# kristi700/ViT-SSL

Hardware: AMD Instinct MI355X
Metric: images_per_sec (higher is better)
Workload: dtype bf16; 1 GPU; ViT-B/16 SimMIM 224x224 mask 0.6 dropout 0.1 AdamW, batch 256/GPU; global_batch=256, parallelism=dp1

## Files before the change

__graft_entry__.py:

```python
import os
import subprocess
import sys
from concurrent.futures import ThreadPoolExecutor

ROOT = os.path.dirname(os.path.abspath(__file__))
PKG = os.path.join(ROOT, "vit-ssl_amd")
CSRC = os.path.join(PKG, "csrc")
OUT_DIR = os.path.join(PKG, "vitssl_hip")
LIB = os.path.join(OUT_DIR, "libvitssl_hip.so")
SOURCES = ["error.cpp", "gemm_nt.hip", "gemm_tn.hip", "layernorm.hip", "attention.hip", "attention_hd.hip", "elementwise.hip", "patch.hip", "dino.hip", "augment.hip", "transforms.hip", "metrics.hip", "classify.hip", "mixup.hip", "fp8.hip", "optim.hip", "droppath.hip", "layerscale.hip", "lamb.hip"]
HIPCC = os.environ.get("HIPCC", "/opt/rocm/bin/hipcc")
PER_FILE_FLAGS = {"augment.hip": ["-ffp-contract=off"], "transforms.hip": ["-ffp-contract=off"]}
FLAGS = ["--offload-arch=gfx950", "-O3", "-fPIC", "-std=c++17", "-Wno-unused-result"] + os.environ.get("VITSSL_HIPCC_FLAGS", "").split()


def _needs_rebuild(target, deps):
    if not os.path.exists(target):
        return True
    t = os.path.getmtime(target)
    return any(os.path.getmtime(d) > t for d in deps if os.path.exists(d))


def build(force: bool = False, verbose: bool = False) -> None:
    srcs = [os.path.join(CSRC, s) for s in SOURCES if os.path.exists(os.path.join(CSRC, s))]
    hdrs = [os.path.join(CSRC, "common.h"), os.path.join(CSRC, "attention_tiles.h"), os.path.join(CSRC, "attention_bwd.h"),
            os.path.join(CSRC, "resample_taps.h"),
            os.path.join(ROOT, "include", "vitssl_hip.h"), os.path.join(ROOT, "include", "vitssl_transforms.h"),
            os.path.join(ROOT, "include", "vitssl_metrics.h"), os.path.join(ROOT, "include", "vitssl_classify.h"),
            os.path.join(ROOT, "include", "vitssl_attention_hd.h"), os.path.join(ROOT, "include", "vitssl_patch.h"),
            os.path.join(ROOT, "include", "vitssl_optim.h"), os.path.join(ROOT, "include", "vitssl_mixup.h"),
            os.path.join(ROOT, "include", "vitssl_droppath.h"), os.path.join(ROOT, "include", "vitssl_layerscale.h"),
            os.path.join(ROOT, "include", "vitssl_lamb.h"), os.path.join(ROOT, "include", "vitssl_bce.h")]
    objdir = os.path.join(CSRC, "build")
    os.makedirs(objdir, exist_ok=True)

    def compile_one(src):
        obj = os.path.join(objdir, os.path.basename(src) + ".o")
        if force or _needs_rebuild(obj, [src] + hdrs + [os.path.abspath(__file__)]):
            cmd = [HIPCC] + FLAGS + PER_FILE_FLAGS.get(os.path.basename(src), []) + ["-x", "hip", "-c", src, "-o", obj]
            r = subprocess.run(cmd, capture_output=True, text=True)
            if r.returncode != 0:
                raise RuntimeError(f"hipcc failed for {src}:\n{r.stderr[-4000:]}")
            if verbose and r.stderr.strip():
                print(r.stderr, file=sys.stderr)
        return obj

    with ThreadPoolExecutor(max_workers=4) as ex:
        objs = list(ex.map(compile_one, srcs))
    if force or _needs_rebuild(LIB, objs):
# ... 24 lines not shown
```

vit-ssl_amd/csrc/gemm_tn.hip:

```cpp
#include <stdlib.h>
#include <type_traits>
#include "common.h"

#ifdef VITSSL_TN_STAMPS
__device__ unsigned long long* g_tn_stamps = nullptr;
extern "C" int vitssl_debug_set_tn_stamps(unsigned long long* p) {
  return hipMemcpyToSymbol(HIP_SYMBOL(g_tn_stamps), &p, sizeof(p)) == hipSuccess ? 0 : 1;
}
#endif

namespace {

constexpr int TN_T = 256;
constexpr int TN_KM = 64;
constexpr int TN8_KM = 128;
constexpr int TN_THREADS = 512;
constexpr int TN_TILE_BYTES = TN_KM * TN_T * 2;
constexpr int TN_LDS_BYTES = 4 * TN_TILE_BYTES;

struct TnPtr {
  const void* p;
  __host__ __device__ operator const bf16_t*() const { return (const bf16_t*)p; }
  __host__ __device__ operator const unsigned char*() const { return (const unsigned char*)p; }
};

struct TnParams {
  TnPtr A, B;
  float* C;
  long long M;
  int N1, N2;
  int tiles1, tiles2, splits;
  int chunks_per_split;
  float* slabs;
  int direct;
  const float* alpha;
  const float* alpha2;
};

// ... 184 lines not shown
    return;
  }
#pragma unroll
  for (int i = 0; i < 8; ++i) {
    const int n1 = c1 + w1 * 128 + i * 16 + (lane & 15);
    if (n1 >= p.N1) continue;
#pragma unroll
    for (int j = 0; j < 4; ++j) {
      const int n2 = c2 + w2 * 64 + j * 16 + 4 * (lane >> 4);
      if (n2 >= p.N2) continue;
      float* q = p.dst + (long long)n1 * p.N2 + n2;
      if (p.mode == 0) {
        *(f32x4*)q = acc[i][j];
      } else if (p.mode == 1) {
        *(f32x4*)q = *(const f32x4*)q + acc[i][j];
      } else {
#pragma unroll
        for (int r = 0; r < 4; ++r) unsafeAtomicAdd(q + r, acc[i][j][r]);
      }
    }
  }
}

constexpr int TN_MAX_JOBS = 8;
struct TnBatchParams {
  const void* A[TN_MAX_JOBS];
  const void* B[TN_MAX_JOBS];
  float* C[TN_MAX_JOBS];
  int N1[TN_MAX_JOBS], N2[TN_MAX_JOBS];
  int tiles2[TN_MAX_JOBS];
  int tile0[TN_MAX_JOBS + 1];
  int njobs;
  long long M;
  int splits, chunks_per_split;
  int rem_chunks;
  float* slots;
};

struct TnBatchWalk {
  int first, step, end;
};
__device__ __forceinline__ TnBatchWalk tn_batch_walk(const TnBatchParams& p) {
  const int G = gridDim.x;
  const int bid = xcd_remap(blockIdx.x, G);
  const int T = p.tile0[p.njobs];
  const int mainu = T * p.splits;
  TnBatchWalk w;
  if (p.rem_chunks > 0) {
    if (bid < mainu) {
      w.first = bid;
      w.step = mainu + T;
      w.end = mainu;
    } else {
      w.first = mainu + (bid - mainu);
      w.step = G - mainu;
      w.end = mainu + T;
    }
  } else {
    w.first = bid;
    w.step = G;
    w.end = mainu;
  }
  return w;
}
__device__ __forceinline__ void tn_batch_unit(const TnBatchParams& p, int un, int km, int& j, int& c1, int& c2, long long& ch_begin, int& nk) {
  const int T = p.tile0[p.njobs];
  const int split = un / T;
  const int gt = un - split * T;
  j = 0;
#pragma unroll
  for (int q = 1; q < TN_MAX_JOBS; ++q)
    if (q < p.njobs && gt >= p.tile0[q]) j = q;
  const int lt = gt - p.tile0[j];
  const int t1 = lt / p.tiles2[j], t2 = lt - t1 * p.tiles2[j];
  c1 = t1 * TN_T;
  c2 = t2 * TN_T;
  const long long total_chunks = (p.M + km - 1) / km;
  ch_begin = (long long)split * p.chunks_per_split;
  long long ch_end = split < p.splits ? ch_begin + p.chunks_per_split : total_chunks;
  if (ch_end > total_chunks) ch_end = total_chunks;
  nk = ch_begin < ch_end ? (int)(ch_end - ch_begin) : 0;
}

struct Tn8BatchParams {
  TnBatchParams b;
  const float* alpha[TN_MAX_JOBS];
  const float* alpha2[TN_MAX_JOBS];
};
template <class P>
__host__ __device__ __forceinline__ auto& tn_base(P& pp) {
  if constexpr (std::is_same_v<std::remove_const_t<P>, Tn8BatchParams>) return pp.b;
  else return pp;
}
__device__ __forceinline__ void tn_job_scalars(const TnBatchParams&, int, TnUnit& u) { u.alpha = u.alpha2 = nullptr; }
__device__ __forceinline__ void tn_job_scalars(const Tn8BatchParams& p, int j, TnUnit& u) {
  u.alpha = p.alpha[j];
  u.alpha2 = p.alpha2[j];
}

__global__ __launch_bounds__(256) void tn_batch_reduce_kernel(TnBatchParams p) {
  const int T = p.tile0[p.njobs];
  const int gt = blockIdx.x >> 3, rblk = blockIdx.x & 7;
  int j = 0;
  for (int q = 1; q < p.njobs; ++q)
    if (gt >= p.tile0[q]) j = q;
  const int lt = gt - p.tile0[j];
  const int t1 = lt / p.tiles2[j], t2 = lt - t1 * p.tiles2[j];
  const int col = 4 * (threadIdx.x & 63);
  const int n2 = t2 * TN_T + col;
  if (n2 >= p.N2[j]) return;
#pragma unroll 2
  for (int r = threadIdx.x >> 6; r < 32; r += 4) {
    const int row = rblk * 32 + r;
    const int n1 = t1 * TN_T + row;
    if (n1 >= p.N1[j]) break;
    float* q = p.C[j] + (long long)n1 * p.N2[j] + n2;
    f32x4 a = *(const f32x4*)q;
    const float* sl = p.slots + (long long)gt * (TN_T * TN_T) + row * TN_T + col;
    const long long sstride = (long long)T * (TN_T * TN_T);
    const int nsl = p.splits + (p.rem_chunks > 0 ? 1 : 0);
    int s = 0;
    for (; s + 4 <= nsl; s += 4) {
      const f32x4 v0 = *(const f32x4*)(sl + (s + 0) * sstride), v1 = *(const f32x4*)(sl + (s + 1) * sstride);
      const f32x4 v2 = *(const f32x4*)(sl + (s + 2) * sstride), v3 = *(const f32x4*)(sl + (s + 3) * sstride);
      a += (v0 + v1) + (v2 + v3);
    }
    for (; s < nsl; ++s) a += *(const f32x4*)(sl + s * sstride);
    *(f32x4*)q = a;
  }
}

__device__ __forceinline__ int tn8_f(int row) { return (row & 7) | (((row >> 5) & 1) << 3); }

__device__ __forceinline__ int tn8_fa(int row) { return ((row >> 1) & 3) | (((row >> 5) & 1) << 2); }

__device__ __forceinline__ void tn8_pp_unit(const TnUnit& p, char* smem) {
  constexpr int AG = TN8_KM * 128;
  constexpr int BT = TN8_KM * 256;
  constexpr int B_BASE = 4 * AG;
  constexpr unsigned OOBV = 0x80000000u;
  const int lane = threadIdx.x & 63;
  const int wave = __builtin_amdgcn_readfirstlane(threadIdx.x >> 6);
  const int w1 = wave >> 2, w2 = wave & 3;
  const int c1 = p.c1, c2 = p.c2;
  const long long ch_begin = p.ch_begin;
  const int nk = p.nk;

  auto window = [&](const unsigned char* base, int ncols, int t) {
    const long long row0 = (ch_begin + t) * (long long)TN8_KM;
    const long long rows = t < nk ? p.M - row0 : 0;
    return __builtin_amdgcn_make_buffer_rsrc((void*)(base + row0 * ncols), 0, (int)(rows * ncols), 0x00020000);
  };
// ... 207 lines not shown
  F::unit(u, smem);
  F::hand_over();
}

__global__ __launch_bounds__(TN_THREADS, 2) void gemm_tn_pp_kernel(TnParams p) {
  extern __shared__ __attribute__((aligned(16))) char smem[];
  tn_single_body<TnBf16>(p, smem);
}
__global__ __launch_bounds__(TN_THREADS, 2) void gemm_tn_fp8_kernel(TnParams p) {
  extern __shared__ __attribute__((aligned(16))) char smem[];
  tn_single_body<TnFp8>(p, smem);
}
__global__ __launch_bounds__(TN_THREADS, 2) void gemm_tn_batch_kernel(TnBatchParams p) {
  extern __shared__ __attribute__((aligned(16))) char smem[];
  const TnBatchWalk w = tn_batch_walk(tn_base(p));
  for (int un = w.first; un < w.end; un += w.step) tn_batch_step<TnBf16>(p, un, smem);
}
__global__ __launch_bounds__(TN_THREADS, 2) void gemm_tn_fp8_batch_kernel(Tn8BatchParams p) {
  extern __shared__ __attribute__((aligned(16))) char smem[];
  const TnBatchWalk w = tn_batch_walk(tn_base(p));
  for (int un = w.first; un < w.end; un += w.step) tn_batch_step<TnFp8>(p, un, smem);
}

__global__ void tn_reduce_kernel(float* __restrict__ C, const float* __restrict__ slabs, long long n4, long long stride, int splits) {
  for (long long i = (long long)blockIdx.x * blockDim.x + threadIdx.x; i < n4; i += (long long)gridDim.x * blockDim.x) {
    f32x4 a = *(const f32x4*)(C + 4 * i);
    for (int s = 0; s < splits; ++s) a += *(const f32x4*)(slabs + s * stride + 4 * i);
    *(f32x4*)(C + 4 * i) = a;
  }
}

int tn_reduce_slabs(float* C, const float* slabs, int N1, int N2, int splits, hipStream_t s, const char* who) {
  const long long n4 = (long long)N1 * N2 / 4;
  long long grid = (n4 + 255) / 256;
  if (grid > 2048) grid = 2048;
  hipLaunchKernelGGL(tn_reduce_kernel, dim3((unsigned)grid), dim3(256), 0, s, C, slabs, n4, (long long)N1 * N2, splits);
  VS_CHECK_LAUNCH(who);
  return VITSSL_OK;
}

void tn_plan(long long M, int N1, int N2, int* tiles1, int* tiles2, int* splits, int* chunks_per_split, int km = TN_KM) {
  *tiles1 = (N1 + TN_T - 1) / TN_T;
  *tiles2 = (N2 + TN_T - 1) / TN_T;
  const long long total_chunks = (M + km - 1) / km;
  const int ntiles = *tiles1 * *tiles2;
  long long sp = vitssl_persistent_cus() / ntiles;
  if (sp < 1) sp = 1;
  if (sp > total_chunks) sp = total_chunks;
  *chunks_per_split = (int)((total_chunks + sp - 1) / sp);
  *splits = (int)((total_chunks + *chunks_per_split - 1) / *chunks_per_split);
}

void tn_batch_plan(long long M, int T, int G, int* splits, int* chunks_per_split, int* rem_chunks, int km = TN_KM) {
  const long long total_chunks = (M + km - 1) / km;
  const double c_kt = 1.46, c_unit = 9.0, c_part = 0.15;
  double best = 1e30;
  int best_s = 1;
  const long long smax = total_chunks < 64 ? total_chunks : 64;
  for (long long sp = 1; sp <= smax; ++sp) {
    const long long cps = (total_chunks + sp - 1) / sp;
    const long long s_eff = (total_chunks + cps - 1) / cps;
    if (s_eff != sp) continue;
    const long long units = (long long)T * sp;
    const long long rounds = (units + G - 1) / G;
    const double cost = (double)rounds * ((double)cps * c_kt + c_unit) + (sp > 1 ? (double)units * c_part : 0.0);
    if (cost < best) {
      best = cost;
      best_s = (int)sp;
    }
  }
  static VsEnvInt forced_env;
  const int forced = forced_env.get("VITSSL_TN_BATCH_SPLITS", 0);
  if (forced > 0 && forced <= total_chunks) best_s = forced;
  *chunks_per_split = (int)((total_chunks + best_s - 1) / best_s);
  *splits = (int)((total_chunks + *chunks_per_split - 1) / *chunks_per_split);
  *rem_chunks = 0;
  static VsEnvInt rem_env;
  const int use_rem = rem_env.get("VITSSL_TN_BATCH_REM", 1);
  const long long mainu = (long long)T * *splits;
  const long long R = G - mainu;
  if (use_rem && mainu <= G && R >= 8) {
    const double c_rem = 2.2;
    const long long S = *splits;
    const double nr = (double)((T + R - 1) / R);
    const double L = (nr * ((double)total_chunks * c_rem + c_unit) - c_unit) / (c_kt + nr * (double)S * c_rem);
    long long Li = (long long)(L + 0.999);
    const long long rem = total_chunks - S * Li;
    const double t_main = (double)Li * c_kt + c_unit, t_rem = nr * ((double)rem * c_rem + c_unit);
    const double t_old = (double)*chunks_per_split * c_kt + c_unit;
    const double tax = (double)T * c_part * (S == 1 ? 2.0 : 1.0);
    if (rem >= 4 && Li >= 4 && (t_main > t_rem ? t_main : t_rem) + tax < 0.95 * t_old) {
      *chunks_per_split = (int)Li;
      *rem_chunks = (int)rem;
    }
  }
}
long long tn_batch_need(int splits, int rem_chunks, int T) {
  return (splits > 1 || rem_chunks > 0) ? (long long)(splits + (rem_chunks > 0)) * T * TN_T * TN_T : 0;
}

void tn_fill_operands(TnBatchParams& p, int j, const vitssl_tn_job_t* q) {
  p.A[j] = q ? q->A : nullptr;
  p.B[j] = q ? q->B : nullptr;
}
void tn_fill_operands(Tn8BatchParams& p, int j, const vitssl_fp8_tn_job_t* q) {
  p.b.A[j] = q ? q->A8 : nullptr;
  p.b.B[j] = q ? q->B8 : nullptr;
  p.alpha[j] = q ? q->alpha : nullptr;
  p.alpha2[j] = q ? q->alpha2 : nullptr;
}
template <class Params, class Job>
int tn_batch_fill(const Job* jobs, int njobs, Params* pp) {
  TnBatchParams& p = tn_base(*pp);
  int t = 0;
  for (int j = 0; j < TN_MAX_JOBS; ++j) {
    const Job* q = j < njobs ? jobs + j : nullptr;
    tn_fill_operands(*pp, j, q);
    p.C[j] = q ? q->C : nullptr;
    p.N1[j] = q ? q->N1 : 0;
    p.N2[j] = q ? q->N2 : 0;
    p.tile0[j] = t;
// ... 3 lines not shown
  p.tile0[TN_MAX_JOBS] = t;
  p.njobs = njobs;
  return t;
}

template <class F>
int tn_check_operands(const void* A, const void* B, const float* C, long long M, int N1, int N2, int job) {
  char who[48];
  if (job < 0) snprintf(who, sizeof who, "%s", F::NAME);
  else snprintf(who, sizeof who, "%s: job %d", F::BATCH, job);
  VS_CHECK_ARG(A && B && C, "%s: null operand", who);
  VS_CHECK_ARG(job >= 0 || (M > 0 && N1 > 0 && N2 > 0), "%s: empty problem", who);
  VS_CHECK_ARG(N1 > 0 && N2 > 0 && N1 % F::COLS == 0 && N2 % F::COLS == 0, "%s: N1=%d N2=%d must be %smultiples of %d", who, N1, N2,
               job < 0 ? "" : "positive ", F::COLS);
  VS_CHECK_ARG((unsigned long long)M * N1 * F::ESZ < (1ull << 31) && (unsigned long long)M * N2 * F::ESZ < (1ull << 31),
               "%s: operand larger than 2 GiB", who);
  return VITSSL_OK;
}

template <class F>
int64_t tn_single_workspace(int64_t M, int N1, int N2) {
  if (M <= 0 || N1 <= 0 || N2 <= 0) return 0;
  int t1, t2, sp, cps;
  tn_plan(M, N1, N2, &t1, &t2, &sp, &cps, F::KM);
  return (int64_t)sp * N1 * N2;
}

template <class F, void (*KERNEL)(TnParams)>
int tn_launch_single(const void* A, const void* B, float* C, int64_t M, int N1, int N2, const float* alpha, const float* alpha2,
                     float* workspace, int64_t workspace_floats, void* stream) {
  if (int rc = tn_check_operands<F>(A, B, C, M, N1, N2, -1)) return rc;
  TnParams p;
  p.A = {A};
  p.B = {B};
  p.C = C;
  p.M = M;
  p.N1 = N1;
  p.N2 = N2;
  p.alpha = alpha;
  p.alpha2 = alpha2;
  tn_plan(M, N1, N2, &p.tiles1, &p.tiles2, &p.splits, &p.chunks_per_split, F::KM);
  const long long need = (long long)p.splits * N1 * N2;
  p.slabs = (workspace && workspace_floats >= need) ? workspace : nullptr;
  VS_CHECK_ARG(!workspace || p.slabs, "%s: workspace too small (%lld < %lld floats, vitssl_%s_workspace_floats)", F::NAME,
               (long long)workspace_floats, need, F::NAME);
  p.direct = p.splits == 1;
  if (p.direct) p.slabs = nullptr;
  static VsOnce attr_done{false};
  if (int rc = ensure_lds(KERNEL, TN_LDS_BYTES, attr_done, F::NAME)) return rc;
  hipStream_t s = (hipStream_t)stream;
  hipLaunchKernelGGL(KERNEL, dim3(p.tiles1 * p.tiles2 * p.splits), dim3(TN_THREADS), TN_LDS_BYTES, s, p);
  VS_CHECK_LAUNCH(F::NAME);
  return p.slabs ? tn_reduce_slabs(C, p.slabs, N1, N2, p.splits, s, F::REDUCE) : VITSSL_OK;
}

template <class F, class Job>
int64_t tn_batch_workspace(const Job* jobs, int njobs, int64_t M) {
  if (!jobs || njobs <= 0 || njobs > TN_MAX_JOBS || M <= 0) return 0;
  typename F::BatchParams pp;
  const int T = tn_batch_fill(jobs, njobs, &pp);
  int sp, cps, rem;
  tn_batch_plan(M, T, vitssl_persistent_cus(), &sp, &cps, &rem, F::KM);
  return tn_batch_need(sp, rem, T);
}

template <class F, void (*KERNEL)(typename F::BatchParams), class Job>
int tn_launch_batch(const Job* jobs, int njobs, int64_t M, float* workspace, int64_t workspace_floats, void* stream) {
  VS_CHECK_ARG(jobs && njobs > 0 && njobs <= TN_MAX_JOBS, "%s: 1..%d jobs", F::BATCH, TN_MAX_JOBS);
  VS_CHECK_ARG(M > 0, "%s: empty problem", F::BATCH);
  typename F::BatchParams pp;
  TnBatchParams& p = tn_base(pp);
  const int T = tn_batch_fill(jobs, njobs, &pp);
  for (int j = 0; j < njobs; ++j)
    if (int rc = tn_check_operands<F>(p.A[j], p.B[j], p.C[j], M, p.N1[j], p.N2[j], j)) return rc;
  p.M = M;
  const long long cus = vitssl_persistent_cus();
  tn_batch_plan(M, T, (int)cus, &p.splits, &p.chunks_per_split, &p.rem_chunks, F::KM);
  const long long need = tn_batch_need(p.splits, p.rem_chunks, T);
  VS_CHECK_ARG(need == 0 || (workspace && workspace_floats >= need), "%s: workspace of %lld floats needed with %lld CUs available (vitssl_%s_workspace_floats; the answer\n"
               "changes with vitssl_set_reserved_cus: query again after changing the reserve)", F::BATCH, need, cus, F::BATCH);
  p.slots = need ? workspace : nullptr;
  static VsOnce attr_done{false};
  if (int rc = ensure_lds(KERNEL, TN_LDS_BYTES, attr_done, F::BATCH)) return rc;
  hipStream_t s = (hipStream_t)stream;
  const long long units = (long long)T * p.splits;
  const unsigned grid = (unsigned)((units < cus && p.rem_chunks == 0) ? units : cus);
  hipLaunchKernelGGL(KERNEL, dim3(grid), dim3(TN_THREADS), TN_LDS_BYTES, s, pp);
  VS_CHECK_LAUNCH(F::BATCH);
  if (p.slots) {
    hipLaunchKernelGGL(tn_batch_reduce_kernel, dim3((unsigned)T * 8u), dim3(256), 0, s, p);
    VS_CHECK_LAUNCH(F::BATCH_REDUCE);
  }
  return VITSSL_OK;
}

}

extern "C" int64_t vitssl_gemm_tn_workspace_floats(int64_t M, int N1, int N2) { return tn_single_workspace<TnBf16>(M, N1, N2); }
extern "C" int64_t vitssl_gemm_fp8_tn_workspace_floats(int64_t M, int N1, int N2) { return tn_single_workspace<TnFp8>(M, N1, N2); }

extern "C" int vitssl_gemm_bf16_tn(const void* A, const void* B, float* C, int64_t M, int N1, int N2, float* workspace,
                                   int64_t workspace_floats, void* stream) {
  return tn_launch_single<TnBf16, gemm_tn_pp_kernel>(A, B, C, M, N1, N2, nullptr, nullptr, workspace, workspace_floats, stream);
}
extern "C" int vitssl_gemm_fp8_tn(const void* A8, const void* B8, float* C, int64_t M, int N1, int N2, const float* alpha,
                                  const float* alpha2, float* workspace, int64_t workspace_floats, void* stream) {
  return tn_launch_single<TnFp8, gemm_tn_fp8_kernel>(A8, B8, C, M, N1, N2, alpha, alpha2, workspace, workspace_floats, stream);
}

extern "C" int64_t vitssl_gemm_tn_batch_workspace_floats(const vitssl_tn_job_t* jobs, int njobs, int64_t M) {
  return tn_batch_workspace<TnBf16>(jobs, njobs, M);
}
extern "C" int64_t vitssl_gemm_fp8_tn_batch_workspace_floats(const vitssl_fp8_tn_job_t* jobs, int njobs, int64_t M) {
  return tn_batch_workspace<TnFp8>(jobs, njobs, M);
}

extern "C" int vitssl_gemm_bf16_tn_batch(const vitssl_tn_job_t* jobs, int njobs, int64_t M, float* workspace, int64_t workspace_floats,
                                         void* stream) {
  return tn_launch_batch<TnBf16, gemm_tn_batch_kernel>(jobs, njobs, M, workspace, workspace_floats, stream);
}
extern "C" int vitssl_gemm_fp8_tn_batch(const vitssl_fp8_tn_job_t* jobs, int njobs, int64_t M, float* workspace, int64_t workspace_floats,
                                        void* stream) {
  return tn_launch_batch<TnFp8, gemm_tn_fp8_batch_kernel>(jobs, njobs, M, workspace, workspace_floats, stream);
}
```

vit-ssl_amd/vitssl_hip/engine.py:

```python
from __future__ import annotations

import re
from typing import Callable, Dict, List, Optional, Tuple

import torch
from torch import nn

from . import _lib as L
from . import ops

BF16 = torch.bfloat16
F32 = torch.float32
FP8 = ops.FP8
ALIGN = 64
MAX_TOKENS = 2048
FP8_MAX_TOKENS = 256

import os as _os

_LINEAR_OPERANDS = _os.environ.get("VITSSL_LINEAR_OPERANDS", "bf16")


def set_linear_operands(kind: str):
    global _LINEAR_OPERANDS
# ... 540 lines not shown
            if save:
                rec["blocks"].append(dict(xin=cur, h1=h1, mean1=mean1, rstd1=rstd1, qkv=qkv, att=att, lse=lse, xmid=xmid,
                                          h2=h2, mean2=mean2, rstd2=rstd2, u=u, a=a))
                if self.fp8:
                    rec["blocks"][-1].update(h1_8=h1_8, att8=att8, h2_8=h2_8, a8=a8)
                if self.layer_scale:
                    rec["blocks"][-1].update(ls1=ls1, ls2=ls2)
            cur = xout
        if save:
            self._saved[slot] = rec
        return cur, probs

    def backward(self, g: torch.Tensor, slot: str = "a", reducer: Optional[GradReducer] = None,
                 scale_key: Optional[str] = None, input_grad_only: bool = False) -> torch.Tensor:
        if self.fp8:
            return self._backward_fp8(g, slot, reducer, scale_key or slot)
        st, D, H, F, dh = self.store, self.D, self.H, self.F, self.dh
        rec = self._saved[slot]
        B, T, seed, training = rec["B"], rec["T"], rec["seed"], rec["training"]
        M = B * T
        dev = g.device
        w = self.ws.get
        bw = f"bwd{M}."
        gm = w(bw + "gm", (M, D), BF16, dev)
        du = w(bw + "du", (M, F), BF16, dev)
        dh_ = w(bw + "dh", (M, D), BF16, dev)
        dqkv = w(bw + "dqkv", (M, 3 * D), BF16, dev)
        delta = w(bw + "delta", (B, H, T), F32, dev)
        gv = st.gview
        last = self.L - 1
        batch = _os.environ.get("VITSSL_TN_BATCH", "1") != "0"
        wgrad = not input_grad_only
        dp = rec.get("dp")
        rows = lambda i, br: (dp[2 * i + br], T) if dp is not None and self.drop_path[i] > 0.0 else None
        gm2 = w(bw + "gm2", (M, D), BF16, dev) if batch and wgrad else gm

        def ls(i, k):
            if not self.layer_scale:
                return {}
            name = self._n(i, f"layer_scale{k}.gamma")
            if not wgrad:
                return dict(cols=st.view(name))
            return dict(cols=st.view(name), branch=rec["blocks"][i][f"ls{k}"], dls=gv(name))

        ops.grad_mask_cast(g, gm, gv(self._n(last, "feed_forward.linear_out.bias")), self._drop(last, 2, seed, training),
                           rows=rows(last, 1), **ls(last, 2))
        for i in range(last, -1, -1):
            s = rec["blocks"][i]
            a_ = self.bp[i] + "self_attention."
            wgrads = [(gm, s["a"], gv(self._n(i, "feed_forward.linear_out.weight"), (D, F))),
                      (du, s["h2"], gv(self._n(i, "feed_forward.linear_in.weight"), (F, D))),
                      (gm2, s["att"], gv(a_ + "final_linear.weight", (D, D))),
                      (dqkv, s["h1"], st.span_view(a_ + "w_query.weight", a_ + "w_value.weight", (3 * D, D), grad=True))]
            ops.gemm_nt(gm, st.w(self._n(i, "w2") + ".T"), du, L.EPI_DGELU, aux=s["u"],
                        colsum=gv(self._n(i, "feed_forward.linear_in.bias")))
            if wgrad and not batch:
                ops.gemm_tn(*wgrads[0])
            ops.gemm_nt(du, st.w(self._n(i, "w1") + ".T"), dh_, L.EPI_BF16)
            if wgrad and not batch:
                ops.gemm_tn(*wgrads[1])
            ops.layernorm_bwd(dh_, s["xmid"], s["mean2"], s["rstd2"], st.view(self._n(i, "layer_norm2.weight")), g, g, gm2,
                              gv(self._n(i, "layer_norm2.weight")), gv(self._n(i, "layer_norm2.bias")), None,
                              self._drop(i, 0, seed, training), rows=rows(i, 0), **ls(i, 1))
            ops.gemm_nt(gm2, st.w(self._n(i, "wo") + ".T"), dh_, L.EPI_BF16)
            if wgrad and not batch:
                ops.gemm_tn(*wgrads[2])
            ops.attn_bwd_any(s["qkv"], s["att"], dh_, s["lse"], dqkv, delta, B, T, H, dh)
            ops.gemm_nt(dqkv, st.w(self._n(i, "wqkv") + ".T"), dh_, L.EPI_BF16)
            if wgrad and batch:
                ops.gemm_tn_batch(wgrads)
            elif wgrad:
                ops.gemm_tn(*wgrads[3])
            if i > 0:
                ops.layernorm_bwd(dh_, s["xin"], s["mean1"], s["rstd1"], st.view(self._n(i, "layer_norm1.weight")), g, g, gm,
                                  gv(self._n(i, "layer_norm1.weight")), gv(self._n(i, "layer_norm1.bias")),
                                  gv(self._n(i - 1, "feed_forward.linear_out.bias")), self._drop(i - 1, 2, seed, training),
                                  rows=rows(i - 1, 1), **ls(i - 1, 2))
            else:
                ops.layernorm_bwd(dh_, s["xin"], s["mean1"], s["rstd1"], st.view(self._n(i, "layer_norm1.weight")), g, g, None,
                                  gv(self._n(i, "layer_norm1.weight")), gv(self._n(i, "layer_norm1.bias")), None, ops.NO_DROP)
            if reducer is not None and wgrad:
                lo, hi = self.block_span(i)
                reducer.ready(lo, hi)
        return g

    @staticmethod
    def _scale_from_amax(amax: torch.Tensor, margin: int) -> torch.Tensor:
        mant, e = torch.frexp(amax)
        k = (9 - e - (mant > 0.875).to(e.dtype) - margin).clamp(-120, 120)
        return torch.bitwise_left_shift(k.to(torch.int32) + 127, 23).view(torch.float32)

    def _grad_scale_state(self, dev, slot: str = "a"):
        gs = self._gs_by_slot.get(slot)
        if gs is None or gs["scale"].device != dev:
            mk = lambda v: torch.full((self.L, 4), v, dtype=F32, device=dev)
            gs = {"scale": mk(1.0), "inv": mk(1.0), "amax": mk(0.0), "used": mk(1.0), "valid": False}
            self._gs_by_slot[slot] = gs
# ... 99 lines not shown
```

vit-ssl_amd/vitssl_hip/ops.py:

```python
import collections
import ctypes as C
import operator

import torch

from . import _lib as L
from ._lib import Dropout, Embed, Fp8Gemm, Gemm, call

BF16 = torch.bfloat16
F32 = torch.float32
FP8 = torch.float8_e4m3fn


def _stream():
    return C.c_void_p(torch.cuda.current_stream().cuda_stream)


def _chk(t, dtype, name, shape=None):
    if t is None:
        raise L.VitsslError(f"{name}: tensor is None")
    if not t.is_cuda:
        raise L.VitsslError(f"{name}: expected a CUDA (HIP) tensor, got {t.device}; there is no CPU fallback")
    if t.device.index != torch.cuda.current_device():
        raise L.VitsslError(f"{name}: tensor lives on {t.device} but the current device is cuda:{torch.cuda.current_device()}; "
# ... 233 lines not shown
    if epilogue == L.EPI_RESID:
        g.aux = _chk(aux, F32, "aux(residual)", (M, N))
    elif epilogue == L.EPI_DGELU:
        g.aux = _chk(aux, BF16, "aux(g')", (M, N))
    g.out1 = _opt(out1, BF16, "out1", (M, N))
    g.colsum = _opt(colsum, F32, "colsum", (N,))
    if colsum is not None:
        g.workspace, g.workspace_floats = _sum_ws(colsum.device, M, N)
    g.drop = drop
    q = Fp8Gemm()
    q.alpha = _scalar(alpha, "alpha")
    q.alpha2 = _scalar(alpha2, "alpha2")
    q.out_fp8 = _opt(out_fp8, FP8, "out_fp8", (M, N))
    q.out_scale = _scalar(out_scale, "out_scale")
    q.out_amax = _scalar(out_amax, "out_amax")
    if out_fp8 is not None and epilogue not in (L.EPI_GELU, L.EPI_DGELU):
        raise L.VitsslError("gemm_fp8_nt: out_fp8 belongs to EPI_GELU / EPI_DGELU")
    ev = _prof_begin()
    call("vitssl_gemm_fp8_nt", C.byref(g), C.byref(q), _stream())
    _prof_end(ev, f"gemm_fp8_nt[epi{epilogue}] {M}x{N}x{K}", 2.0 * M * N * K)


_TN_WS = {}


def _tn_workspace(device, floats):
    key = (device, torch.cuda.current_stream().cuda_stream)
    ws = _TN_WS.get(key)
    if ws is None or ws.numel() < floats:
        ws = torch.empty(max(floats, 1 << 20), dtype=F32, device=device)
        _TN_WS[key] = ws
    return ws


def _sum_ws(device, rows, cols):
    ws = _tn_workspace(device, int(L.lib().vitssl_sum_workspace_floats(rows, cols)))
    return C.c_void_p(ws.data_ptr()), ws.numel()


_TnKind = collections.namedtuple("_TnKind", "label dtype sfx scalars entry query batch_entry batch_query Job")
_TN_BF16 = _TnKind("gemm_tn", BF16, "", (), "vitssl_gemm_bf16_tn", "vitssl_gemm_tn_workspace_floats",
                   "vitssl_gemm_bf16_tn_batch", "vitssl_gemm_tn_batch_workspace_floats", L.TnJob)
_TN_FP8 = _TnKind("gemm_fp8_tn", FP8, "8", ("alpha", "alpha2"), "vitssl_gemm_fp8_tn", "vitssl_gemm_fp8_tn_workspace_floats",
                  "vitssl_gemm_fp8_tn_batch", "vitssl_gemm_fp8_tn_batch_workspace_floats", L.Fp8TnJob)


# ... 612 lines not shown
```

Measured before the change: 7693 images/s.

## Add list-based TN weight-grad batching with body/tail split and deferred multi-block batching

Adds a list-driven batched TN GEMM kernel that takes an arbitrary job table. Whole tiles fill full persistent-CU waves as a non-split body, and only the leftover tail is split along K and reduced through slots. The engine can optionally defer weight-gradient GEMMs across several blocks into one launch, using rotating per-block gradient buffers. The aim is to cut launch count and wave quantization in the backward weight-gradient pass, at the cost of extra workspace memory and a binary search over the job table. The deferral is gated behind an environment variable that is off by default.

Result: no change. 7690 images/s, median of 2 (-0.0%).

```diff
diff --git a/__graft_entry__.py b/__graft_entry__.py
--- a/__graft_entry__.py
+++ b/__graft_entry__.py
@@ -24,7 +24,7 @@
 def build(force: bool = False, verbose: bool = False) -> None:
     srcs = [os.path.join(CSRC, s) for s in SOURCES if os.path.exists(os.path.join(CSRC, s))]
     hdrs = [os.path.join(CSRC, "common.h"), os.path.join(CSRC, "attention_tiles.h"), os.path.join(CSRC, "attention_bwd.h"),
-            os.path.join(CSRC, "resample_taps.h"),
+            os.path.join(CSRC, "resample_taps.h"), os.path.join(CSRC, "tn_plan.h"),
             os.path.join(ROOT, "include", "vitssl_hip.h"), os.path.join(ROOT, "include", "vitssl_transforms.h"),
             os.path.join(ROOT, "include", "vitssl_metrics.h"), os.path.join(ROOT, "include", "vitssl_classify.h"),
             os.path.join(ROOT, "include", "vitssl_attention_hd.h"), os.path.join(ROOT, "include", "vitssl_patch.h"),
diff --git a/vit-ssl_amd/csrc/gemm_tn.hip b/vit-ssl_amd/csrc/gemm_tn.hip
--- a/vit-ssl_amd/csrc/gemm_tn.hip
+++ b/vit-ssl_amd/csrc/gemm_tn.hip
@@ -1,6 +1,7 @@
 #include <stdlib.h>
 #include <type_traits>
 #include "common.h"
+#include "tn_plan.h"
 
 #ifdef VITSSL_TN_STAMPS
 __device__ unsigned long long* g_tn_stamps = nullptr;
@@ -11,9 +12,6 @@
 
 namespace {
 
-constexpr int TN_T = 256;
-constexpr int TN_KM = 64;
-constexpr int TN8_KM = 128;
 constexpr int TN_THREADS = 512;
 constexpr int TN_TILE_BYTES = TN_KM * TN_T * 2;
 constexpr int TN_LDS_BYTES = 4 * TN_TILE_BYTES;
@@ -244,7 +242,6 @@
   }
 }
 
-constexpr int TN_MAX_JOBS = 8;
 struct TnBatchParams {
   const void* A[TN_MAX_JOBS];
   const void* B[TN_MAX_JOBS];
@@ -259,31 +256,9 @@
   float* slots;
 };
 
-struct TnBatchWalk {
-  int first, step, end;
-};
 __device__ __forceinline__ TnBatchWalk tn_batch_walk(const TnBatchParams& p) {
   const int G = gridDim.x;
-  const int bid = xcd_remap(blockIdx.x, G);
-  const int T = p.tile0[p.njobs];
-  const int mainu = T * p.splits;
-  TnBatchWalk w;
-  if (p.rem_chunks > 0) {
-    if (bid < mainu) {
-      w.first = bid;
-      w.step = mainu + T;
-      w.end = mainu;
-    } else {
-      w.first = mainu + (bid - mainu);
-      w.step = G - mainu;
-      w.end = mainu + T;
-    }
-  } else {
-    w.first = bid;
-    w.step = G;
-    w.end = mainu;
-  }
-  return w;
+  return tn_walk_units(xcd_remap(blockIdx.x, G), G, p.tile0[p.njobs], p.splits, p.rem_chunks);
 }
 __device__ __forceinline__ void tn_batch_unit(const TnBatchParams& p, int un, int km, int& j, int& c1, int& c2, long long& ch_begin, int& nk) {
   const int T = p.tile0[p.njobs];
@@ -320,6 +295,28 @@
   u.alpha2 = p.alpha2[j];
 }
 
+__device__ __forceinline__ void tn_reduce_rows(float* C, int N1, int N2, int t1, int t2, int rblk, const float* sl, long long sstride, int nsl) {
+  const int col = 4 * (threadIdx.x & 63);
+  const int n2 = t2 * TN_T + col;
+  if (n2 >= N2) return;
+#pragma unroll 2
+  for (int r = threadIdx.x >> 6; r < 32; r += 4) {
+    const int row = rblk * 32 + r;
+    const int n1 = t1 * TN_T + row;
+    if (n1 >= N1) break;
+    float* q = C + (long long)n1 * N2 + n2;
+    f32x4 a = *(const f32x4*)q;
+    const float* slr = sl + row * TN_T + col;
+    int s = 0;
+    for (; s + 4 <= nsl; s += 4) {
+      const f32x4 v0 = *(const f32x4*)(slr + (s + 0) * sstride), v1 = *(const f32x4*)(slr + (s + 1) * sstride);
+      const f32x4 v2 = *(const f32x4*)(slr + (s + 2) * sstride), v3 = *(const f32x4*)(slr + (s + 3) * sstride);
+      a += (v0 + v1) + (v2 + v3);
+    }
+    for (; s < nsl; ++s) a += *(const f32x4*)(slr + s * sstride);
+    *(f32x4*)q = a;
+  }
+}
 __global__ __launch_bounds__(256) void tn_batch_reduce_kernel(TnBatchParams p) {
   const int T = p.tile0[p.njobs];
   const int gt = blockIdx.x >> 3, rblk = blockIdx.x & 7;
@@ -328,28 +325,50 @@
     if (gt >= p.tile0[q]) j = q;
   const int lt = gt - p.tile0[j];
   const int t1 = lt / p.tiles2[j], t2 = lt - t1 * p.tiles2[j];
-  const int col = 4 * (threadIdx.x & 63);
-  const int n2 = t2 * TN_T + col;
-  if (n2 >= p.N2[j]) return;
-#pragma unroll 2
-  for (int r = threadIdx.x >> 6; r < 32; r += 4) {
-    const int row = rblk * 32 + r;
-    const int n1 = t1 * TN_T + row;
-    if (n1 >= p.N1[j]) break;
-    float* q = p.C[j] + (long long)n1 * p.N2[j] + n2;
-    f32x4 a = *(const f32x4*)q;
-    const float* sl = p.slots + (long long)gt * (TN_T * TN_T) + row * TN_T + col;
-    const long long sstride = (long long)T * (TN_T * TN_T);
-    const int nsl = p.splits + (p.rem_chunks > 0 ? 1 : 0);
-    int s = 0;
-    for (; s + 4 <= nsl; s += 4) {
-      const f32x4 v0 = *(const f32x4*)(sl + (s + 0) * sstride), v1 = *(const f32x4*)(sl + (s + 1) * sstride);
-      const f32x4 v2 = *(const f32x4*)(sl + (s + 2) * sstride), v3 = *(const f32x4*)(sl + (s + 3) * sstride);
-      a += (v0 + v1) + (v2 + v3);
-    }
-    for (; s < nsl; ++s) a += *(const f32x4*)(sl + s * sstride);
-    *(f32x4*)q = a;
-  }
+  tn_reduce_rows(p.C[j], p.N1[j], p.N2[j], t1, t2, rblk, p.slots + (long long)gt * (TN_T * TN_T), (long long)T * (TN_T * TN_T),
+                 p.splits + (p.rem_chunks > 0 ? 1 : 0));
+}
+
+struct TnListJob {
+  const void *A, *B;
+  float* C;
+  const float *alpha, *alpha2;
+  int N1, N2;
+  int tiles2, tile0;
+};
+struct TnListParams {
+  const TnListJob* jobs;
+  int njobs;
+  long long M;
+  int body, tail;
+  int splits, chunks_per_split, rem_chunks;
+  float* slots;
+};
+__device__ __forceinline__ int tn_uniform(int v) { return __builtin_amdgcn_readfirstlane(v); }
+template <class T>
+__device__ __forceinline__ T* tn_uniform(T* q) {
+  const unsigned long long v = (unsigned long long)q;
+  return (T*)(((unsigned long long)(unsigned)tn_uniform((int)(v >> 32)) << 32) | (unsigned)tn_uniform((int)v));
+}
+__device__ __forceinline__ TnListJob tn_list_job(const TnListParams& p, int gt) {
+  int lo = 0, hi = p.njobs - 1;
+  while (lo < hi) {
+    const int mid = (lo + hi + 1) >> 1;
+    if (tn_uniform(p.jobs[mid].tile0) <= gt) lo = mid;
+    else hi = mid - 1;
+  }
+  const TnListJob& q = p.jobs[lo];
+  return {tn_uniform(q.A), tn_uniform(q.B), tn_uniform(q.C), tn_uniform(q.alpha), tn_uniform(q.alpha2),
+          tn_uniform(q.N1), tn_uniform(q.N2), tn_uniform(q.tiles2), tn_uniform(q.tile0)};
+}
+__global__ __launch_bounds__(256) void tn_list_reduce_kernel(TnListParams p) {
+  const int tt = blockIdx.x >> 3, rblk = blockIdx.x & 7;
+  const int gt = p.body + tt;
+  const TnListJob q = tn_list_job(p, gt);
+  const int lt = gt - q.tile0;
+  const int t1 = lt / q.tiles2, t2 = lt - t1 * q.tiles2;
+  tn_reduce_rows(q.C, q.N1, q.N2, t1, t2, rblk, p.slots + (long long)tt * (TN_T * TN_T), (long long)p.tail * (TN_T * TN_T),
+                 p.splits + (p.rem_chunks > 0 ? 1 : 0));
 }
 
 __device__ __forceinline__ int tn8_f(int row) { return (row & 7) | (((row >> 5) & 1) << 3); }
@@ -603,6 +622,58 @@
   for (int un = w.first; un < w.end; un += w.step) tn_batch_step<TnFp8>(p, un, smem);
 }
 
+template <class F>
+__device__ __forceinline__ void tn_list_body(const TnListParams& p, char* smem) {
+  const int G = gridDim.x;
+  const int bid = xcd_remap(blockIdx.x, G);
+  const long long total_chunks = (p.M + F::KM - 1) / F::KM;
+  const TnBatchWalk w = tn_walk_units(bid, G, p.tail, p.splits, p.rem_chunks);
+  int gt = bid, un = w.first;
+  for (;;) {
+    TnUnit u;
+    int tile;
+    if (gt < p.body) {
+      tile = gt;
+      gt += G;
+      u.ch_begin = 0;
+      u.nk = (int)total_chunks;
+      u.dst = nullptr;
+    } else if (un < w.end) {
+      tn_unit_range(un, p.tail, p.splits, p.chunks_per_split, total_chunks, tile, u.ch_begin, u.nk);
+      tile += p.body;
+      u.dst = p.slots ? p.slots + (long long)un * (TN_T * TN_T) : nullptr;
+      un += w.step;
+    } else {
+      break;
+    }
+    const TnListJob q = tn_list_job(p, tile);
+    const int lt = tile - q.tile0;
+    const int t1 = lt / q.tiles2, t2 = lt - t1 * q.tiles2;
+    u.A = {q.A};
+    u.B = {q.B};
+    u.M = p.M;
+    u.N1 = q.N1;
+    u.N2 = q.N2;
+    u.c1 = t1 * TN_T;
+    u.c2 = t2 * TN_T;
+    u.mode = u.dst ? 3 : 1;
+    if (!u.dst) u.dst = q.C;
+    u.alpha = q.alpha;
+    u.alpha2 = q.alpha2;
+    u.stamp_wg = -1;
+    F::unit(u, smem);
+    F::hand_over();
+  }
+}
+__global__ __launch_bounds__(TN_THREADS, 2) void gemm_tn_list_kernel(TnListParams p) {
+  extern __shared__ __attribute__((aligned(16))) char smem[];
+  tn_list_body<TnBf16>(p, smem);
+}
+__global__ __launch_bounds__(TN_THREADS, 2) void gemm_tn_fp8_list_kernel(TnListParams p) {
+  extern __shared__ __attribute__((aligned(16))) char smem[];
+  tn_list_body<TnFp8>(p, smem);
+}
+
 __global__ void tn_reduce_kernel(float* __restrict__ C, const float* __restrict__ slabs, long long n4, long long stride, int splits) {
   for (long long i = (long long)blockIdx.x * blockDim.x + threadIdx.x; i < n4; i += (long long)gridDim.x * blockDim.x) {
     f32x4 a = *(const f32x4*)(C + 4 * i);
@@ -620,64 +691,13 @@
   return VITSSL_OK;
 }
 
-void tn_plan(long long M, int N1, int N2, int* tiles1, int* tiles2, int* splits, int* chunks_per_split, int km = TN_KM) {
-  *tiles1 = (N1 + TN_T - 1) / TN_T;
-  *tiles2 = (N2 + TN_T - 1) / TN_T;
-  const long long total_chunks = (M + km - 1) / km;
-  const int ntiles = *tiles1 * *tiles2;
-  long long sp = vitssl_persistent_cus() / ntiles;
-  if (sp < 1) sp = 1;
-  if (sp > total_chunks) sp = total_chunks;
-  *chunks_per_split = (int)((total_chunks + sp - 1) / sp);
-  *splits = (int)((total_chunks + *chunks_per_split - 1) / *chunks_per_split);
-}
-
-void tn_batch_plan(long long M, int T, int G, int* splits, int* chunks_per_split, int* rem_chunks, int km = TN_KM) {
-  const long long total_chunks = (M + km - 1) / km;
-  const double c_kt = 1.46, c_unit = 9.0, c_part = 0.15;
-  double best = 1e30;
-  int best_s = 1;
-  const long long smax = total_chunks < 64 ? total_chunks : 64;
-  for (long long sp = 1; sp <= smax; ++sp) {
-    const long long cps = (total_chunks + sp - 1) / sp;
-    const long long s_eff = (total_chunks + cps - 1) / cps;
-    if (s_eff != sp) continue;
-    const long long units = (long long)T * sp;
-    const long long rounds = (units + G - 1) / G;
-    const double cost = (double)rounds * ((double)cps * c_kt + c_unit) + (sp > 1 ? (double)units * c_part : 0.0);
-    if (cost < best) {
-      best = cost;
-      best_s = (int)sp;
-    }
-  }
-  static VsEnvInt forced_env;
-  const int forced = forced_env.get("VITSSL_TN_BATCH_SPLITS", 0);
-  if (forced > 0 && forced <= total_chunks) best_s = forced;
-  *chunks_per_split = (int)((total_chunks + best_s - 1) / best_s);
-  *splits = (int)((total_chunks + *chunks_per_split - 1) / *chunks_per_split);
-  *rem_chunks = 0;
-  static VsEnvInt rem_env;
-  const int use_rem = rem_env.get("VITSSL_TN_BATCH_REM", 1);
-  const long long mainu = (long long)T * *splits;
-  const long long R = G - mainu;
-  if (use_rem && mainu <= G && R >= 8) {
-    const double c_rem = 2.2;
-    const long long S = *splits;
-    const double nr = (double)((T + R - 1) / R);
-    const double L = (nr * ((double)total_chunks * c_rem + c_unit) - c_unit) / (c_kt + nr * (double)S * c_rem);
-    long long Li = (long long)(L + 0.999);
-    const long long rem = total_chunks - S * Li;
-    const double t_main = (double)Li * c_kt + c_unit, t_rem = nr * ((double)rem * c_rem + c_unit);
-    const double t_old = (double)*chunks_per_split * c_kt + c_unit;
-    const double tax = (double)T * c_part * (S == 1 ? 2.0 : 1.0);
-    if (rem >= 4 && Li >= 4 && (t_main > t_rem ? t_main : t_rem) + tax < 0.95 * t_old) {
-      *chunks_per_split = (int)Li;
-      *rem_chunks = (int)rem;
-    }
-  }
-}
-long long tn_batch_need(int splits, int rem_chunks, int T) {
-  return (splits > 1 || rem_chunks > 0) ? (long long)(splits + (rem_chunks > 0)) * T * TN_T * TN_T : 0;
+TnPlanKnobs tn_knobs() {
+  static VsEnvInt forced_env, rem_env, tail_env;
+  TnPlanKnobs k;
+  k.forced_splits = forced_env.get("VITSSL_TN_BATCH_SPLITS", 0);
+  k.use_rem = rem_env.get("VITSSL_TN_BATCH_REM", 1);
+  k.use_tail = tail_env.get("VITSSL_TN_BATCH_TAIL", 1);
+  return k;
 }
 
 void tn_fill_operands(TnBatchParams& p, int j, const vitssl_tn_job_t* q) {
@@ -727,7 +747,7 @@
 int64_t tn_single_workspace(int64_t M, int N1, int N2) {
   if (M <= 0 || N1 <= 0 || N2 <= 0) return 0;
   int t1, t2, sp, cps;
-  tn_plan(M, N1, N2, &t1, &t2, &sp, &cps, F::KM);
+  tn_plan(M, N1, N2, vitssl_persistent_cus(), &t1, &t2, &sp, &cps, F::KM);
   return (int64_t)sp * N1 * N2;
 }
 
@@ -744,7 +764,7 @@
   p.N2 = N2;
   p.alpha = alpha;
   p.alpha2 = alpha2;
-  tn_plan(M, N1, N2, &p.tiles1, &p.tiles2, &p.splits, &p.chunks_per_split, F::KM);
+  tn_plan(M, N1, N2, vitssl_persistent_cus(), &p.tiles1, &p.tiles2, &p.splits, &p.chunks_per_split, F::KM);
   const long long need = (long long)p.splits * N1 * N2;
   p.slabs = (workspace && workspace_floats >= need) ? workspace : nullptr;
   VS_CHECK_ARG(!workspace || p.slabs, "%s: workspace too small (%lld < %lld floats, vitssl_%s_workspace_floats)", F::NAME,
@@ -759,41 +779,115 @@
   return p.slabs ? tn_reduce_slabs(C, p.slabs, N1, N2, p.splits, s, F::REDUCE) : VITSSL_OK;
 }
 
+constexpr long long TN_MAX_LIST_TILES = 1 << 24;
+void tn_row_operands(TnListJob& r, const vitssl_tn_job_t& q) {
+  r.A = q.A;
+  r.B = q.B;
+  r.alpha = r.alpha2 = nullptr;
+}
+void tn_row_operands(TnListJob& r, const vitssl_fp8_tn_job_t& q) {
+  r.A = q.A8;
+  r.B = q.B8;
+  r.alpha = q.alpha;
+  r.alpha2 = q.alpha2;
+}
+template <class Job>
+long long tn_list_fill(const Job* jobs, int njobs, TnListJob* rows) {
+  long long t = 0;
+  for (int j = 0; j < njobs; ++j) {
+    TnListJob& r = rows[j];
+    tn_row_operands(r, jobs[j]);
+    r.C = jobs[j].C;
+    r.N1 = jobs[j].N1;
+    r.N2 = jobs[j].N2;
+    r.tiles2 = (r.N2 + TN_T - 1) / TN_T;
+    r.tile0 = (int)t;
+    if (r.N1 > 0 && r.N2 > 0) t += (long long)((r.N1 + TN_T - 1) / TN_T) * r.tiles2;
+  }
+  return t;
+}
+bool tn_short_list(int njobs) { return njobs <= TN_MAX_JOBS; }
+TnListPlan tn_plan_list(int njobs, long long M, int T, int G, int km) {
+  if (!tn_short_list(njobs)) return tn_list_plan(M, T, G, km, tn_knobs());
+  TnListPlan pl;
+  pl.body = 0;
+  pl.tail = T;
+  tn_batch_plan(M, T, G, &pl.splits, &pl.chunks_per_split, &pl.rem_chunks, km, tn_knobs());
+  return pl;
+}
+long long tn_table_floats(int njobs) {
+  return ((long long)njobs * (long long)sizeof(TnListJob) + 255) / 256 * 64;
+}
+
 template <class F, class Job>
 int64_t tn_batch_workspace(const Job* jobs, int njobs, int64_t M) {
-  if (!jobs || njobs <= 0 || njobs > TN_MAX_JOBS || M <= 0) return 0;
-  typename F::BatchParams pp;
-  const int T = tn_batch_fill(jobs, njobs, &pp);
-  int sp, cps, rem;
-  tn_batch_plan(M, T, vitssl_persistent_cus(), &sp, &cps, &rem, F::KM);
-  return tn_batch_need(sp, rem, T);
-}
-
-template <class F, void (*KERNEL)(typename F::BatchParams), class Job>
+  if (!jobs || njobs <= 0 || njobs > TN_MAX_LIST_JOBS || M <= 0) return 0;
+  TnListJob rows[TN_MAX_LIST_JOBS];
+  const long long T = tn_list_fill(jobs, njobs, rows);
+  if (T <= 0 || T > TN_MAX_LIST_TILES) return 0;
+  const int cus = vitssl_persistent_cus();
+  const TnListPlan pl = tn_plan_list(njobs, M, (int)T, cus, F::KM);
+  return tn_list_need(pl) + (tn_short_list(njobs) ? 0 : tn_table_floats(njobs));
+}
+
+template <class F, void (*KERNEL)(typename F::BatchParams), void (*LIST_KERNEL)(TnListParams), class Job>
 int tn_launch_batch(const Job* jobs, int njobs, int64_t M, float* workspace, int64_t workspace_floats, void* stream) {
-  VS_CHECK_ARG(jobs && njobs > 0 && njobs <= TN_MAX_JOBS, "%s: 1..%d jobs", F::BATCH, TN_MAX_JOBS);
+  VS_CHECK_ARG(jobs && njobs > 0 && njobs <= TN_MAX_LIST_JOBS, "%s: 1..%d jobs", F::BATCH, TN_MAX_LIST_JOBS);
   VS_CHECK_ARG(M > 0, "%s: empty problem", F::BATCH);
-  typename F::BatchParams pp;
-  TnBatchParams& p = tn_base(pp);
-  const int T = tn_batch_fill(jobs, njobs, &pp);
+  TnListJob rows[TN_MAX_LIST_JOBS];
+  const long long T = tn_list_fill(jobs, njobs, rows);
   for (int j = 0; j < njobs; ++j)
-    if (int rc = tn_check_operands<F>(p.A[j], p.B[j], p.C[j], M, p.N1[j], p.N2[j], j)) return rc;
-  p.M = M;
+    if (int rc = tn_check_operands<F>(rows[j].A, rows[j].B, rows[j].C, M, rows[j].N1, rows[j].N2, j)) return rc;
+  VS_CHECK_ARG(T <= TN_MAX_LIST_TILES, "%s: more than %lld tiles in one list", F::BATCH, TN_MAX_LIST_TILES);
   const long long cus = vitssl_persistent_cus();
-  tn_batch_plan(M, T, (int)cus, &p.splits, &p.chunks_per_split, &p.rem_chunks, F::KM);
-  const long long need = tn_batch_need(p.splits, p.rem_chunks, T);
+  const TnListPlan pl = tn_plan_list(njobs, M, (int)T, (int)cus, F::KM);
+  const bool short_list = tn_short_list(njobs);
+  const long long table = short_list ? 0 : tn_table_floats(njobs);
+  const long long need = tn_list_need(pl) + table;
   VS_CHECK_ARG(need == 0 || (workspace && workspace_floats >= need), "%s: workspace of %lld floats needed with %lld CUs available (vitssl_%s_workspace_floats; the answer\n"
                "changes with vitssl_set_reserved_cus: query again after changing the reserve)", F::BATCH, need, cus, F::BATCH);
-  p.slots = need ? workspace : nullptr;
-  static VsOnce attr_done{false};
-  if (int rc = ensure_lds(KERNEL, TN_LDS_BYTES, attr_done, F::BATCH)) return rc;
   hipStream_t s = (hipStream_t)stream;
-  const long long units = (long long)T * p.splits;
-  const unsigned grid = (unsigned)((units < cus && p.rem_chunks == 0) ? units : cus);
-  hipLaunchKernelGGL(KERNEL, dim3(grid), dim3(TN_THREADS), TN_LDS_BYTES, s, pp);
+  const unsigned grid = tn_list_grid(pl, (int)cus);
+  if (short_list) {
+    typename F::BatchParams pp;
+    TnBatchParams& p = tn_base(pp);
+    tn_batch_fill(jobs, njobs, &pp);
+    p.M = M;
+    p.splits = pl.splits;
+    p.chunks_per_split = pl.chunks_per_split;
+    p.rem_chunks = pl.rem_chunks;
+    p.slots = need ? workspace : nullptr;
+    static VsOnce attr_done{false};
+    if (int rc = ensure_lds(KERNEL, TN_LDS_BYTES, attr_done, F::BATCH)) return rc;
+    hipLaunchKernelGGL(KERNEL, dim3(grid), dim3(TN_THREADS), TN_LDS_BYTES, s, pp);
+    VS_CHECK_LAUNCH(F::BATCH);
+    if (p.slots) {
+      hipLaunchKernelGGL(tn_batch_reduce_kernel, dim3((unsigned)T * 8u), dim3(256), 0, s, p);
+      VS_CHECK_LAUNCH(F::BATCH_REDUCE);
+    }
+    return VITSSL_OK;
+  }
+  TnListParams p;
+  p.jobs = (const TnListJob*)workspace;
+  p.njobs = njobs;
+  p.M = M;
+  p.body = pl.body;
+  p.tail = pl.tail;
+  p.splits = pl.splits;
+  p.chunks_per_split = pl.chunks_per_split;
+  p.rem_chunks = pl.rem_chunks;
+  p.slots = need > table ? workspace + table : nullptr;
+  static VsOnce list_attr_done{false};
+  if (int rc = ensure_lds(LIST_KERNEL, TN_LDS_BYTES, list_attr_done, F::BATCH)) return rc;
+  const hipError_t e = hipMemcpyAsync(workspace, rows, (size_t)njobs * sizeof(TnListJob), hipMemcpyHostToDevice, s);
+  if (e != hipSuccess) {
+    vitssl_set_error("%s: copy of the job table failed: %s", F::BATCH, hipGetErrorString(e));
+    return VITSSL_ERR_LAUNCH;
+  }
+  hipLaunchKernelGGL(LIST_KERNEL, dim3(grid), dim3(TN_THREADS), TN_LDS_BYTES, s, p);
   VS_CHECK_LAUNCH(F::BATCH);
   if (p.slots) {
-    hipLaunchKernelGGL(tn_batch_reduce_kernel, dim3((unsigned)T * 8u), dim3(256), 0, s, p);
+    hipLaunchKernelGGL(tn_list_reduce_kernel, dim3((unsigned)pl.tail * 8u), dim3(256), 0, s, p);
     VS_CHECK_LAUNCH(F::BATCH_REDUCE);
   }
   return VITSSL_OK;
@@ -822,9 +916,9 @@
 
 extern "C" int vitssl_gemm_bf16_tn_batch(const vitssl_tn_job_t* jobs, int njobs, int64_t M, float* workspace, int64_t workspace_floats,
                                          void* stream) {
-  return tn_launch_batch<TnBf16, gemm_tn_batch_kernel>(jobs, njobs, M, workspace, workspace_floats, stream);
+  return tn_launch_batch<TnBf16, gemm_tn_batch_kernel, gemm_tn_list_kernel>(jobs, njobs, M, workspace, workspace_floats, stream);
 }
 extern "C" int vitssl_gemm_fp8_tn_batch(const vitssl_fp8_tn_job_t* jobs, int njobs, int64_t M, float* workspace, int64_t workspace_floats,
                                         void* stream) {
-  return tn_launch_batch<TnFp8, gemm_tn_fp8_batch_kernel>(jobs, njobs, M, workspace, workspace_floats, stream);
-}
+  return tn_launch_batch<TnFp8, gemm_tn_fp8_batch_kernel, gemm_tn_fp8_list_kernel>(jobs, njobs, M, workspace, workspace_floats, stream);
+}
diff --git a/vit-ssl_amd/csrc/tn_plan.h b/vit-ssl_amd/csrc/tn_plan.h
--- /dev/null
+++ b/vit-ssl_amd/csrc/tn_plan.h
@@ -0,0 +1,132 @@
+#pragma once
+#include <stdint.h>
+
+constexpr int TN_T = 256;
+constexpr int TN_KM = 64;
+constexpr int TN8_KM = 128;
+constexpr int TN_MAX_JOBS = 8;
+constexpr int TN_MAX_LIST_JOBS = 128;
+
+struct TnPlanKnobs {
+  int forced_splits = 0;
+  int use_rem = 1;
+  int use_tail = 1;
+};
+
+inline void tn_plan(long long M, int N1, int N2, int G, int* tiles1, int* tiles2, int* splits, int* chunks_per_split, int km = TN_KM) {
+  *tiles1 = (N1 + TN_T - 1) / TN_T;
+  *tiles2 = (N2 + TN_T - 1) / TN_T;
+  const long long total_chunks = (M + km - 1) / km;
+  const int ntiles = *tiles1 * *tiles2;
+  long long sp = G / ntiles;
+  if (sp < 1) sp = 1;
+  if (sp > total_chunks) sp = total_chunks;
+  *chunks_per_split = (int)((total_chunks + sp - 1) / sp);
+  *splits = (int)((total_chunks + *chunks_per_split - 1) / *chunks_per_split);
+}
+
+inline void tn_batch_plan(long long M, int T, int G, int* splits, int* chunks_per_split, int* rem_chunks, int km = TN_KM,
+                          const TnPlanKnobs& knobs = TnPlanKnobs()) {
+  const long long total_chunks = (M + km - 1) / km;
+  const double c_kt = 1.46, c_unit = 9.0, c_part = 0.15;
+  double best = 1e30;
+  int best_s = 1;
+  const long long smax = total_chunks < 64 ? total_chunks : 64;
+  for (long long sp = 1; sp <= smax; ++sp) {
+    const long long cps = (total_chunks + sp - 1) / sp;
+    const long long s_eff = (total_chunks + cps - 1) / cps;
+    if (s_eff != sp) continue;
+    const long long units = (long long)T * sp;
+    const long long rounds = (units + G - 1) / G;
+    const double cost = (double)rounds * ((double)cps * c_kt + c_unit) + (sp > 1 ? (double)units * c_part : 0.0);
+    if (cost < best) {
+      best = cost;
+      best_s = (int)sp;
+    }
+  }
+  const int forced = knobs.forced_splits;
+  if (forced > 0 && forced <= total_chunks) best_s = forced;
+  *chunks_per_split = (int)((total_chunks + best_s - 1) / best_s);
+  *splits = (int)((total_chunks + *chunks_per_split - 1) / *chunks_per_split);
+  *rem_chunks = 0;
+  const long long mainu = (long long)T * *splits;
+  const long long R = G - mainu;
+  if (knobs.use_rem && mainu <= G && R >= 8) {
+    const double c_rem = 2.2;
+    const long long S = *splits;
+    const double nr = (double)((T + R - 1) / R);
+    const double L = (nr * ((double)total_chunks * c_rem + c_unit) - c_unit) / (c_kt + nr * (double)S * c_rem);
+    long long Li = (long long)(L + 0.999);
+    const long long rem = total_chunks - S * Li;
+    const double t_main = (double)Li * c_kt + c_unit, t_rem = nr * ((double)rem * c_rem + c_unit);
+    const double t_old = (double)*chunks_per_split * c_kt + c_unit;
+    const double tax = (double)T * c_part * (S == 1 ? 2.0 : 1.0);
+    if (rem >= 4 && Li >= 4 && (t_main > t_rem ? t_main : t_rem) + tax < 0.95 * t_old) {
+      *chunks_per_split = (int)Li;
+      *rem_chunks = (int)rem;
+    }
+  }
+}
+inline long long tn_batch_need(int splits, int rem_chunks, int T) {
+  return (splits > 1 || rem_chunks > 0) ? (long long)(splits + (rem_chunks > 0)) * T * TN_T * TN_T : 0;
+}
+
+struct TnListPlan {
+  int body;
+  int tail;
+  int splits, chunks_per_split, rem_chunks;
+};
+inline TnListPlan tn_list_plan(long long M, int T, int G, int km = TN_KM, const TnPlanKnobs& knobs = TnPlanKnobs()) {
+  TnListPlan pl;
+  pl.body = T > G ? (T / G) * G : 0;
+  pl.tail = T - pl.body;
+  const long long total_chunks = (M + km - 1) / km;
+  pl.splits = 1;
+  pl.chunks_per_split = (int)total_chunks;
+  pl.rem_chunks = 0;
+  if (pl.tail > 0 && (pl.body == 0 || knobs.use_tail)) tn_batch_plan(M, pl.tail, G, &pl.splits, &pl.chunks_per_split, &pl.rem_chunks, km, knobs);
+  return pl;
+}
+inline long long tn_list_need(const TnListPlan& pl) { return tn_batch_need(pl.splits, pl.rem_chunks, pl.tail); }
+
+struct TnBatchWalk {
+  int first, step, end;
+};
+#if defined(__HIPCC__)
+#define TN_PLAN_HD __host__ __device__ __forceinline__
+#else
+#define TN_PLAN_HD inline
+#endif
+TN_PLAN_HD TnBatchWalk tn_walk_units(int bid, int G, int T, int splits, int rem_chunks) {
+  const int mainu = T * splits;
+  TnBatchWalk w;
+  if (rem_chunks > 0) {
+    if (bid < mainu) {
+      w.first = bid;
+      w.step = mainu + T;
+      w.end = mainu;
+    } else {
+      w.first = mainu + (bid - mainu);
+      w.step = G - mainu;
+      w.end = mainu + T;
+    }
+  } else {
+    w.first = bid;
+    w.step = G;
+    w.end = mainu;
+  }
+  return w;
+}
+TN_PLAN_HD void tn_unit_range(int un, int T, int splits, int chunks_per_split, long long total_chunks, int& tile, long long& ch_begin, int& nk) {
+  const int split = un / T;
+  tile = un - split * T;
+  ch_begin = (long long)split * chunks_per_split;
+  long long ch_end = split < splits ? ch_begin + chunks_per_split : total_chunks;
+  if (ch_end > total_chunks) ch_end = total_chunks;
+  nk = ch_begin < ch_end ? (int)(ch_end - ch_begin) : 0;
+}
+inline unsigned tn_list_grid(const TnListPlan& pl, int G) {
+  if (pl.body > 0) return (unsigned)G;
+  const long long units = (long long)pl.tail * pl.splits;
+  return (unsigned)((units < G && pl.rem_chunks == 0) ? units : G);
+}
diff --git a/vit-ssl_amd/vitssl_hip/engine.py b/vit-ssl_amd/vitssl_hip/engine.py
--- a/vit-ssl_amd/vitssl_hip/engine.py
+++ b/vit-ssl_amd/vitssl_hip/engine.py
@@ -586,10 +586,7 @@
         dev = g.device
         w = self.ws.get
         bw = f"bwd{M}."
-        gm = w(bw + "gm", (M, D), BF16, dev)
-        du = w(bw + "du", (M, F), BF16, dev)
         dh_ = w(bw + "dh", (M, D), BF16, dev)
-        dqkv = w(bw + "dqkv", (M, 3 * D), BF16, dev)
         delta = w(bw + "delta", (B, H, T), F32, dev)
         gv = st.gview
         last = self.L - 1
@@ -597,7 +594,18 @@
         wgrad = not input_grad_only
         dp = rec.get("dp")
         rows = lambda i, br: (dp[2 * i + br], T) if dp is not None and self.drop_path[i] > 0.0 else None
-        gm2 = w(bw + "gm2", (M, D), BF16, dev) if batch and wgrad else gm
+        k = 1
+        if wgrad and batch and reducer is None and _os.environ.get("VITSSL_TN_DEFER", "0") not in ("", "0"):
+            per_block = M * (2 * D + F + 3 * D) * 2
+            k = int(_os.environ.get("VITSSL_TN_DEFER_BLOCKS", "0")) or (int(_os.environ.get("VITSSL_TN_DEFER_MB", "16384")) << 20) // per_block
+            k = max(1, min(k, self.L, ops.TN_MAX_LIST_JOBS // 4))
+
+        def operands(i):
+            sfx = f".{(last - i) % k}" if k > 1 else ""
+            gm = w(bw + "gm" + sfx, (M, D), BF16, dev)
+            return (gm, w(bw + "du" + sfx, (M, F), BF16, dev), w(bw + "gm2" + sfx, (M, D), BF16, dev) if batch and wgrad else gm,
+                    w(bw + "dqkv" + sfx, (M, 3 * D), BF16, dev))
+        pending = []
 
         def ls(i, k):
             if not self.layer_scale:
@@ -607,11 +615,12 @@
                 return dict(cols=st.view(name))
             return dict(cols=st.view(name), branch=rec["blocks"][i][f"ls{k}"], dls=gv(name))
 
-        ops.grad_mask_cast(g, gm, gv(self._n(last, "feed_forward.linear_out.bias")), self._drop(last, 2, seed, training),
+        ops.grad_mask_cast(g, operands(last)[0], gv(self._n(last, "feed_forward.linear_out.bias")), self._drop(last, 2, seed, training),
                            rows=rows(last, 1), **ls(last, 2))
         for i in range(last, -1, -1):
             s = rec["blocks"][i]
             a_ = self.bp[i] + "self_attention."
+            gm, du, gm2, dqkv = operands(i)
             wgrads = [(gm, s["a"], gv(self._n(i, "feed_forward.linear_out.weight"), (D, F))),
                       (du, s["h2"], gv(self._n(i, "feed_forward.linear_in.weight"), (F, D))),
                       (gm2, s["att"], gv(a_ + "final_linear.weight", (D, D))),
@@ -632,11 +641,14 @@
             ops.attn_bwd_any(s["qkv"], s["att"], dh_, s["lse"], dqkv, delta, B, T, H, dh)
             ops.gemm_nt(dqkv, st.w(self._n(i, "wqkv") + ".T"), dh_, L.EPI_BF16)
             if wgrad and batch:
-                ops.gemm_tn_batch(wgrads)
+                pending += wgrads
+                if i == 0 or (last - i) % k == k - 1:
+                    ops.gemm_tn_batch(pending)
+                    pending = []
             elif wgrad:
                 ops.gemm_tn(*wgrads[3])
             if i > 0:
-                ops.layernorm_bwd(dh_, s["xin"], s["mean1"], s["rstd1"], st.view(self._n(i, "layer_norm1.weight")), g, g, gm,
+                ops.layernorm_bwd(dh_, s["xin"], s["mean1"], s["rstd1"], st.view(self._n(i, "layer_norm1.weight")), g, g, operands(i - 1)[0],
                                   gv(self._n(i, "layer_norm1.weight")), gv(self._n(i, "layer_norm1.bias")),
                                   gv(self._n(i - 1, "feed_forward.linear_out.bias")), self._drop(i - 1, 2, seed, training),
                                   rows=rows(i - 1, 1), **ls(i - 1, 2))
diff --git a/vit-ssl_amd/vitssl_hip/ops.py b/vit-ssl_amd/vitssl_hip/ops.py
--- a/vit-ssl_amd/vitssl_hip/ops.py
+++ b/vit-ssl_amd/vitssl_hip/ops.py
@@ -279,6 +279,7 @@
 
 
 _TN_WS = {}
+TN_MAX_LIST_JOBS = 128
 
 
 def _tn_workspace(device, floats):
```
